# plai-group/latent-flexible-video-diffusion-modeling

Measured on AMD Instinct MI355X. Metric: denoising steps/sec on 20-frame 4x16x16 latents (sampling; training reported alongside), higher is better.
Workload: dtype f32

## Files before the change

### latent-flexible-video-diffusion-modeling_amd/csrc/attention_spatial_fused.hip

```cpp
#include <cstdlib>

#include "common_hip.h"

namespace {

constexpr unsigned kOOBs = 0x40000000u;

__device__ __forceinline__ bool sf_wg(int N, int heads, int& n, int& h) {
    const int L = blockIdx.x;
    const int xcd = L & 7, r = L >> 3;
    const int slot = r / heads;
    h = r - slot * heads;
    n = slot * 8 + xcd;
    return n < N;
}

template <int FP>
__global__ __launch_bounds__(1024) void attn_spatial_fused_kernel(const float* __restrict__ xn, const float* __restrict__ W,
                                                                 const float* __restrict__ bias, float* __restrict__ o,
                                                                 int N, int P, int C, int heads) {
    constexpr int FG = FP / 16;
    constexpr int QLD = FP + 8, VLD = FP + 4;
    extern __shared__ __attribute__((aligned(16))) float sf_smem[];
    int n, h;
    if (!sf_wg(N, heads, n, h)) return;
    const int tid = threadIdx.x, lane = tid & 63;
    const int wave = __builtin_amdgcn_readfirstlane(tid >> 6);
    const int NW = (int)(blockDim.x >> 6);
    const int lq = lane & 15, kk = lane >> 4;
    const int PP = (P + 15) & ~15;
    const int SPR = C >> 2;
    float* Xs = sf_smem;
    float* Ws = Xs + (size_t)PP * C;
    float* Qs = Ws + (size_t)3 * FP * C;
    float* Ks = Qs + (size_t)PP * QLD;
    float* Vs = Ks + (size_t)PP * QLD;

    {
        const __amdgpu_buffer_rsrc_t rsX = __builtin_amdgcn_make_buffer_rsrc((void*)(xn + (size_t)n * P * C), 0, P * C * 4, 0x00020000);
        const __amdgpu_buffer_rsrc_t rsW = __builtin_amdgcn_make_buffer_rsrc((void*)W, 0, 3 * C * C * 4, 0x00020000);
        const int sh = 31 - __builtin_clz(SPR);
        const int nX = (PP * SPR + 63) >> 6, nW = (3 * FP * SPR + 63) >> 6;
        const bool pow2 = (SPR & (SPR - 1)) == 0;
        for (int pc = wave; pc < nX + nW; pc += NW) {
            const bool isX = pc < nX;
            const int ps = (isX ? pc : pc - nX) * 64 + lane;
            int r, s;
            if (pow2) { r = ps >> sh; s = ps & (SPR - 1); }
            else { r = (int)(((float)ps + 0.5f) * __builtin_amdgcn_rcpf((float)SPR)); s = ps - r * SPR; }
            const int ls = (s & ~15) | ((s ^ r) & 15);
            unsigned off;
            if (isX) {
                off = r < P ? (unsigned)(r * C + ls * 4) * 4u : kOOBs;
            } else {
                const int which = r / FP, f = r - which * FP;
                off = r < 3 * FP ? (unsigned)((which * C + h * FP + f) * C + ls * 4) * 4u : kOOBs;
            }
            float* dst = (isX ? Xs : Ws) + (size_t)(isX ? pc : pc - nX) * 256;
            __builtin_amdgcn_raw_ptr_buffer_load_lds(isX ? rsX : rsW, (__attribute__((address_space(3))) void*)dst, 16, (int)off, 0, 0, 0);
        }
    }
    asm volatile("s_waitcnt vmcnt(0)" ::: "memory");
    __syncthreads();

    {
        const float scale = rsqrtf((float)FP) * 1.4426950408889634f;
        const int NRT = PP >> 4;
        const int CG = C >> 4;
        for (int item = wave; item < NRT * FG; item += NW) {
            const int rt = item / FG, fg = item - rt * FG;
            const int xr = 16 * rt + lq;
            const float* xrow = Xs + (size_t)xr * C;
            int wr[3];
            const float* wrow[3];
#pragma unroll
            for (int w = 0; w < 3; ++w) {
                wr[w] = w * FP + 16 * fg + lq;
                wrow[w] = Ws + (size_t)wr[w] * C;
            }
            f32x4 acc[3];
#pragma unroll
            for (int w = 0; w < 3; ++w) acc[w] = (f32x4){0.f, 0.f, 0.f, 0.f};
            for (int g = 0; g < CG; ++g) {
                const int s = 4 * g + kk;
                const f32x4 a4 = ld4(xrow + (((s & ~15) | ((s ^ xr) & 15)) << 2));
                f32x4 b4[3];
#pragma unroll
                for (int w = 0; w < 3; ++w) b4[w] = ld4(wrow[w] + (((s & ~15) | ((s ^ wr[w]) & 15)) << 2));
#pragma unroll
                for (int e = 0; e < 4; ++e)
#pragma unroll
                    for (int w = 0; w < 3; ++w) acc[w] = __builtin_amdgcn_mfma_f32_16x16x4f32(a4[e], b4[w][e], acc[w], 0, 0, 0);
            }
            const int f = 16 * fg + lq;
#pragma unroll
            for (int w = 0; w < 3; ++w) {
                const float bv = bias[w * C + h * FP + f];
                float* dst = w == 0 ? Qs : (w == 1 ? Ks : Vs);
                const int ld = w == 2 ? VLD : QLD;
#pragma unroll
                for (int r = 0; r < 4; ++r) {
                    float v = acc[w][r] + bv;
                    if (w == 0) v *= scale;
                    dst[(size_t)(16 * rt + 4 * kk + r) * ld + f] = v;
                }
            }
        }
    }
    __syncthreads();

    const int NQT = PP >> 4;
    for (int qt = wave; qt < NQT; qt += NW) {
        const int q = 16 * qt + lq;
        f32x4 qf[FG], oacc[FG], oacc2[FG];
#pragma unroll
        for (int g = 0; g < FG; ++g) {
            qf[g] = ld4(Qs + (size_t)q * QLD + 16 * g + 4 * kk);
            oacc[g] = (f32x4){0.f, 0.f, 0.f, 0.f};
            oacc2[g] = (f32x4){0.f, 0.f, 0.f, 0.f};
        }
        float m_run = -INFINITY, l_run = 0.f;
        for (int kb = 0; kb < P; kb += 64) {
            f32x4 s[4];
            int keyr[4];
#pragma unroll
            for (int j = 0; j < 4; ++j) {
                s[j] = (f32x4){0.f, 0.f, 0.f, 0.f};
                keyr[j] = min(kb + 16 * j + lq, PP - 1);
            }
#pragma unroll
            for (int g = 0; g < FG; ++g) {
                f32x4 k4[4];
#pragma unroll
                for (int j = 0; j < 4; ++j) k4[j] = ld4(Ks + (size_t)keyr[j] * QLD + 16 * g + 4 * kk);
#pragma unroll
                for (int e = 0; e < 4; ++e)
#pragma unroll
                    for (int j = 0; j < 4; ++j) s[j] = __builtin_amdgcn_mfma_f32_16x16x4f32(k4[j][e], qf[g][e], s[j], 0, 0, 0);
            }
            float mx = -INFINITY;
            if (kb + 64 > P) {
#pragma unroll
                for (int j = 0; j < 4; ++j)
#pragma unroll
                    for (int r = 0; r < 4; ++r)
                        if (kb + 16 * j + 4 * kk + r >= P) s[j][r] = -INFINITY;
            }
#pragma unroll
            for (int j = 0; j < 4; ++j)
#pragma unroll
                for (int r = 0; r < 4; ++r) mx = fmaxf(mx, s[j][r]);
            mx = fmaxf(mx, __shfl_xor(mx, 16, 64));
            mx = fmaxf(mx, __shfl_xor(mx, 32, 64));
            const float m_new = fmaxf(m_run, mx);
            const float alpha = __builtin_amdgcn_exp2f(m_run - m_new);
            float psum = 0.f;
#pragma unroll
            for (int j = 0; j < 4; ++j)
#pragma unroll
                for (int r = 0; r < 4; ++r) {
                    const float pv = __builtin_amdgcn_exp2f(s[j][r] - m_new);
                    s[j][r] = pv;
                    psum += pv;
                }
            l_run = l_run * alpha + psum;
            m_run = m_new;
#pragma unroll
            for (int g = 0; g < FG; ++g) { oacc[g] *= alpha; oacc2[g] *= alpha; }
#pragma unroll
            for (int j = 0; j < 4; j += 2)
#pragma unroll
                for (int r = 0; r < 4; ++r) {
                    const int key0 = min(kb + 16 * j + 4 * kk + r, PP - 1);
                    const int key1 = min(kb + 16 * (j + 1) + 4 * kk + r, PP - 1);
                    const float* v0 = Vs + (size_t)key0 * VLD + lq;
                    const float* v1 = Vs + (size_t)key1 * VLD + lq;
#pragma unroll
                    for (int g = 0; g < FG; ++g) {
                        oacc[g] = __builtin_amdgcn_mfma_f32_16x16x4f32(v0[16 * g], s[j][r], oacc[g], 0, 0, 0);
                        oacc2[g] = __builtin_amdgcn_mfma_f32_16x16x4f32(v1[16 * g], s[j + 1][r], oacc2[g], 0, 0, 0);
                    }
                }
        }
        l_run += __shfl_xor(l_run, 16, 64);
        l_run += __shfl_xor(l_run, 32, 64);
        const float inv = 1.0f / l_run;
        if (q < P) {
#pragma unroll
            for (int g = 0; g < FG; ++g) st4(o + ((size_t)n * P + q) * C + h * FP + 16 * g + 4 * kk, (oacc[g] + oacc2[g]) * inv);
        }
    }
}

inline size_t sf_lds_bytes(int P, int C, int FP) {
    const size_t PP = (size_t)((P + 15) & ~15);
    const size_t xs = (PP * C + 255) & ~(size_t)255, ws = ((size_t)3 * FP * C + 255) & ~(size_t)255;
    return (xs + ws + 2 * PP * (FP + 8) + PP * (FP + 4)) * sizeof(float);
}

}

extern "C" int lfvdm_attn_spatial_fused_ok(int N, int P, int C, int heads) {
    if (N <= 0 || P <= 0 || heads <= 0 || C % heads) return LFVDM_E_SHAPE;
    const int F = C / heads;
    if ((F != 16 && F != 32 && F != 64) || C % 64) return LFVDM_E_UNSUPPORTED;
    if ((long)P * C * 4 >= (1L << 30) || sf_lds_bytes(P, C, F) > 160 * 1024) return LFVDM_E_UNSUPPORTED;
    return LFVDM_OK;
}

extern "C" int lfvdm_attn_spatial_fused(const float* xn, const float* Wqkv, const float* bqkv, float* o, int N, int P, int C,
                                        int heads, void* stream) {
    if (!xn || !Wqkv || !bqkv || !o) return LFVDM_E_SHAPE;
    if (int rc = lfvdm_attn_spatial_fused_ok(N, P, C, heads)) return rc;
    const int F = C / heads;
    const size_t lds = sf_lds_bytes(P, C, F);
    const unsigned grid = 8u * (unsigned)((N + 7) / 8) * (unsigned)heads;
    const int PP = (P + 15) & ~15, items = (PP / 16) * (F / 16);
    int nw = PP / 16 > items ? PP / 16 : items;
    nw = nw < 4 ? 4 : nw > 16 ? 16 : nw;
    static const int force_nw = getenv("LFVDM_SF_WAVES") ? atoi(getenv("LFVDM_SF_WAVES")) : 0;
    if (force_nw >= 1 && force_nw <= 16) nw = force_nw;
    hipStream_t s = (hipStream_t)stream;
#define LFVDM_SF(FV)                                                                                                         \
    {                                                                                                                        \
        static DynLdsLimit limit;                                                                                            \
        if (int rc = limit.ensure(reinterpret_cast<const void*>(&attn_spatial_fused_kernel<FV>), lds)) return rc;            \
        hipLaunchKernelGGL((attn_spatial_fused_kernel<FV>), dim3(grid), dim3(64 * nw), lds, s, xn, Wqkv, bqkv, o, N, P, C, heads); \
    }
    if (F == 16) LFVDM_SF(16)
    else if (F == 32) LFVDM_SF(32)
    else LFVDM_SF(64)
#undef LFVDM_SF
    LFVDM_CHECK_LAUNCH();
    return LFVDM_OK;
}
```

Baseline: 1231.

## Double-buffer X row chunks in spatial attention QKV projection to overlap loads

The X tile is now staged into LDS in row chunks with two buffers, so the QKV projection of one chunk overlaps the buffer loads of the next, and LDS footprint shrinks. Work items are split per Q/K/V matrix to expose more parallelism, bias values are prefetched into registers, and the K loop is unrolled by four. This adds finer-grained waits and barriers, and changes the wave-count heuristic (minimum of four removed). The extra synchronisation per chunk may cost more than it saves on small spatial sizes.

```diff
diff --git a/latent-flexible-video-diffusion-modeling_amd/csrc/attention_spatial_fused.hip b/latent-flexible-video-diffusion-modeling_amd/csrc/attention_spatial_fused.hip
--- a/latent-flexible-video-diffusion-modeling_amd/csrc/attention_spatial_fused.hip
+++ b/latent-flexible-video-diffusion-modeling_amd/csrc/attention_spatial_fused.hip
@@ -13,6 +13,25 @@
     h = r - slot * heads;
     n = slot * 8 + xcd;
     return n < N;
+}
+
+__host__ __device__ inline int sf_chunk_rows(int C) {
+    const int ch = (4096 / C) & ~15;
+    return ch < 16 ? 16 : ch;
+}
+
+__device__ __forceinline__ void lds_barrier() {
+    asm volatile("s_waitcnt lgkmcnt(0)" ::: "memory");
+    __builtin_amdgcn_s_barrier();
+    asm volatile("" ::: "memory");
+}
+
+__device__ __forceinline__ void sf_wait_vm(int n) {
+    if (n <= 0) asm volatile("s_waitcnt vmcnt(0)" ::: "memory");
+    else if (n == 1) asm volatile("s_waitcnt vmcnt(1)" ::: "memory");
+    else if (n == 2) asm volatile("s_waitcnt vmcnt(2)" ::: "memory");
+    else if (n == 3) asm volatile("s_waitcnt vmcnt(3)" ::: "memory");
+    else asm volatile("s_waitcnt vmcnt(4)" ::: "memory");
 }
 
 template <int FP>
@@ -30,84 +49,110 @@
     const int lq = lane & 15, kk = lane >> 4;
     const int PP = (P + 15) & ~15;
     const int SPR = C >> 2;
+    const int CH = sf_chunk_rows(C);
+    const int NCH = (PP + CH - 1) / CH;
+    const size_t XB = (size_t)CH * C;
     float* Xs = sf_smem;
-    float* Ws = Xs + (size_t)PP * C;
+    float* Ws = Xs + (size_t)(PP < 2 * CH ? PP : 2 * CH) * C;
     float* Qs = Ws + (size_t)3 * FP * C;
     float* Ks = Qs + (size_t)PP * QLD;
     float* Vs = Ks + (size_t)PP * QLD;
 
-    {
-        const __amdgpu_buffer_rsrc_t rsX = __builtin_amdgcn_make_buffer_rsrc((void*)(xn + (size_t)n * P * C), 0, P * C * 4, 0x00020000);
-        const __amdgpu_buffer_rsrc_t rsW = __builtin_amdgcn_make_buffer_rsrc((void*)W, 0, 3 * C * C * 4, 0x00020000);
-        const int sh = 31 - __builtin_clz(SPR);
-        const int nX = (PP * SPR + 63) >> 6, nW = (3 * FP * SPR + 63) >> 6;
-        const bool pow2 = (SPR & (SPR - 1)) == 0;
-        for (int pc = wave; pc < nX + nW; pc += NW) {
-            const bool isX = pc < nX;
-            const int ps = (isX ? pc : pc - nX) * 64 + lane;
+    float bvs[3][FG];
+#pragma unroll
+    for (int w = 0; w < 3; ++w)
+#pragma unroll
+        for (int g = 0; g < FG; ++g)
+            asm volatile("global_load_dword %0, %1, off" : "=&v"(bvs[w][g]) : "v"(bias + w * C + h * FP + 16 * g + lq) : "memory");
+
+    const __amdgpu_buffer_rsrc_t rsX = __builtin_amdgcn_make_buffer_rsrc((void*)(xn + (size_t)n * P * C), 0, P * C * 4, 0x00020000);
+    const int sh = 31 - __builtin_clz(SPR);
+    const bool pow2 = (SPR & (SPR - 1)) == 0;
+    auto chunk_pieces = [&](int c) { return ((PP - c * CH < CH ? PP - c * CH : CH) * SPR) >> 6; };
+    auto my_pieces = [&](int npc) { return wave < npc ? (npc - wave + NW - 1) / NW : 0; };
+    auto stage_chunk = [&](int c) {
+        const int r0 = c * CH, npc = chunk_pieces(c);
+        float* buf = Xs + (size_t)(c & 1) * XB;
+        for (int pc = wave; pc < npc; pc += NW) {
+            const int ps = pc * 64 + lane;
             int r, s;
             if (pow2) { r = ps >> sh; s = ps & (SPR - 1); }
             else { r = (int)(((float)ps + 0.5f) * __builtin_amdgcn_rcpf((float)SPR)); s = ps - r * SPR; }
             const int ls = (s & ~15) | ((s ^ r) & 15);
-            unsigned off;
-            if (isX) {
-                off = r < P ? (unsigned)(r * C + ls * 4) * 4u : kOOBs;
-            } else {
-                const int which = r / FP, f = r - which * FP;
-                off = r < 3 * FP ? (unsigned)((which * C + h * FP + f) * C + ls * 4) * 4u : kOOBs;
-            }
-            float* dst = (isX ? Xs : Ws) + (size_t)(isX ? pc : pc - nX) * 256;
-            __builtin_amdgcn_raw_ptr_buffer_load_lds(isX ? rsX : rsW, (__attribute__((address_space(3))) void*)dst, 16, (int)off, 0, 0, 0);
-        }
-    }
-    asm volatile("s_waitcnt vmcnt(0)" ::: "memory");
-    __syncthreads();
+            const unsigned off = r0 + r < P ? (unsigned)((r0 + r) * C + ls * 4) * 4u : kOOBs;
+            __builtin_amdgcn_raw_ptr_buffer_load_lds(rsX, (__attribute__((address_space(3))) void*)(buf + (size_t)pc * 256), 16, (int)off, 0, 0, 0);
+        }
+    };
+    {
+        const __amdgpu_buffer_rsrc_t rsW = __builtin_amdgcn_make_buffer_rsrc((void*)W, 0, 3 * C * C * 4, 0x00020000);
+        const int nW = (3 * FP * SPR) >> 6;
+        for (int pc = wave; pc < nW; pc += NW) {
+            const int ps = pc * 64 + lane;
+            int r, s;
+            if (pow2) { r = ps >> sh; s = ps & (SPR - 1); }
+            else { r = (int)(((float)ps + 0.5f) * __builtin_amdgcn_rcpf((float)SPR)); s = ps - r * SPR; }
+            const int ls = (s & ~15) | ((s ^ r) & 15);
+            const int which = r / FP, f = r - which * FP;
+            const unsigned off = r < 3 * FP ? (unsigned)((which * C + h * FP + f) * C + ls * 4) * 4u : kOOBs;
+            __builtin_amdgcn_raw_ptr_buffer_load_lds(rsW, (__attribute__((address_space(3))) void*)(Ws + (size_t)pc * 256), 16, (int)off, 0, 0, 0);
+        }
+    }
+    stage_chunk(0);
+    if (NCH > 1) stage_chunk(1);
 
     {
         const float scale = rsqrtf((float)FP) * 1.4426950408889634f;
-        const int NRT = PP >> 4;
         const int CG = C >> 4;
-        for (int item = wave; item < NRT * FG; item += NW) {
-            const int rt = item / FG, fg = item - rt * FG;
-            const int xr = 16 * rt + lq;
-            const float* xrow = Xs + (size_t)xr * C;
-            int wr[3];
-            const float* wrow[3];
-#pragma unroll
-            for (int w = 0; w < 3; ++w) {
-                wr[w] = w * FP + 16 * fg + lq;
-                wrow[w] = Ws + (size_t)wr[w] * C;
-            }
-            f32x4 acc[3];
-#pragma unroll
-            for (int w = 0; w < 3; ++w) acc[w] = (f32x4){0.f, 0.f, 0.f, 0.f};
-            for (int g = 0; g < CG; ++g) {
-                const int s = 4 * g + kk;
-                const f32x4 a4 = ld4(xrow + (((s & ~15) | ((s ^ xr) & 15)) << 2));
-                f32x4 b4[3];
-#pragma unroll
-                for (int w = 0; w < 3; ++w) b4[w] = ld4(wrow[w] + (((s & ~15) | ((s ^ wr[w]) & 15)) << 2));
-#pragma unroll
-                for (int e = 0; e < 4; ++e)
-#pragma unroll
-                    for (int w = 0; w < 3; ++w) acc[w] = __builtin_amdgcn_mfma_f32_16x16x4f32(a4[e], b4[w][e], acc[w], 0, 0, 0);
-            }
-            const int f = 16 * fg + lq;
-#pragma unroll
-            for (int w = 0; w < 3; ++w) {
-                const float bv = bias[w * C + h * FP + f];
+        for (int c = 0; c < NCH; ++c) {
+            sf_wait_vm(c == 0 && NCH > 1 ? my_pieces(chunk_pieces(1)) : 0);
+#pragma unroll
+            for (int w = 0; w < 3; ++w)
+#pragma unroll
+                for (int g = 0; g < FG; ++g) asm volatile("" : "+v"(bvs[w][g]));
+            lds_barrier();
+            if (c >= 1 && c + 1 < NCH) stage_chunk(c + 1);
+            const int rows = PP - c * CH < CH ? PP - c * CH : CH;
+            const float* buf = Xs + (size_t)(c & 1) * XB;
+            for (int item = wave; item < (rows >> 4) * 3 * FG; item += NW) {
+                const int rtl = item / (3 * FG), t = item - rtl * 3 * FG;
+                const int fg = t / 3, w = t - 3 * fg;
+                const int xr = 16 * rtl + lq;
+                const float* xrow = buf + (size_t)xr * C;
+                const int wr = w * FP + 16 * fg + lq;
+                const float* wrow = Ws + (size_t)wr * C;
+                f32x4 acc = (f32x4){0.f, 0.f, 0.f, 0.f};
+                for (int g4 = 0; g4 < CG; g4 += 4) {
+                    f32x4 a4[4], b4[4];
+#pragma unroll
+                    for (int u = 0; u < 4; ++u) {
+                        const int s = 4 * (g4 + u) + kk;
+                        a4[u] = ld4(xrow + (((s & ~15) | ((s ^ xr) & 15)) << 2));
+                        b4[u] = ld4(wrow + (((s & ~15) | ((s ^ wr) & 15)) << 2));
+                    }
+#pragma unroll
+                    for (int u = 0; u < 4; ++u)
+#pragma unroll
+                        for (int e = 0; e < 4; ++e) acc = __builtin_amdgcn_mfma_f32_16x16x4f32(a4[u][e], b4[u][e], acc, 0, 0, 0);
+                }
+                const int f = 16 * fg + lq;
+                float bv = 0.f;
+#pragma unroll
+                for (int w2 = 0; w2 < 3; ++w2)
+#pragma unroll
+                    for (int g2 = 0; g2 < FG; ++g2)
+                        if (w2 == w && g2 == fg) bv = bvs[w2][g2];
                 float* dst = w == 0 ? Qs : (w == 1 ? Ks : Vs);
                 const int ld = w == 2 ? VLD : QLD;
 #pragma unroll
                 for (int r = 0; r < 4; ++r) {
-                    float v = acc[w][r] + bv;
+                    float v = acc[r] + bv;
                     if (w == 0) v *= scale;
-                    dst[(size_t)(16 * rt + 4 * kk + r) * ld + f] = v;
-                }
-            }
-        }
-    }
-    __syncthreads();
+                    dst[(size_t)(c * CH + 16 * rtl + 4 * kk + r) * ld + f] = v;
+                }
+            }
+        }
+    }
+    lds_barrier();
 
     const int NQT = PP >> 4;
     for (int qt = wave; qt < NQT; qt += NW) {
@@ -193,6 +238,12 @@
 }
 
 inline size_t sf_lds_bytes(int P, int C, int FP) {
+    const size_t PP = (size_t)((P + 15) & ~15), CH = (size_t)sf_chunk_rows(C);
+    const size_t xs = (PP < 2 * CH ? PP : 2 * CH) * C, ws = (size_t)3 * FP * C;
+    return (xs + ws + 2 * PP * (FP + 8) + PP * (FP + 4)) * sizeof(float);
+}
+
+inline size_t sf_admit_bytes(int P, int C, int FP) {
     const size_t PP = (size_t)((P + 15) & ~15);
     const size_t xs = (PP * C + 255) & ~(size_t)255, ws = ((size_t)3 * FP * C + 255) & ~(size_t)255;
     return (xs + ws + 2 * PP * (FP + 8) + PP * (FP + 4)) * sizeof(float);
@@ -204,7 +255,7 @@
     if (N <= 0 || P <= 0 || heads <= 0 || C % heads) return LFVDM_E_SHAPE;
     const int F = C / heads;
     if ((F != 16 && F != 32 && F != 64) || C % 64) return LFVDM_E_UNSUPPORTED;
-    if ((long)P * C * 4 >= (1L << 30) || sf_lds_bytes(P, C, F) > 160 * 1024) return LFVDM_E_UNSUPPORTED;
+    if ((long)P * C * 4 >= (1L << 30) || sf_admit_bytes(P, C, F) > 160 * 1024) return LFVDM_E_UNSUPPORTED;
     return LFVDM_OK;
 }
 
@@ -215,9 +266,10 @@
     const int F = C / heads;
     const size_t lds = sf_lds_bytes(P, C, F);
     const unsigned grid = 8u * (unsigned)((N + 7) / 8) * (unsigned)heads;
-    const int PP = (P + 15) & ~15, items = (PP / 16) * (F / 16);
+    const int PP = (P + 15) & ~15, CH = sf_chunk_rows(C);
+    const int items = ((PP < CH ? PP : CH) / 16) * 3 * (F / 16);
     int nw = PP / 16 > items ? PP / 16 : items;
-    nw = nw < 4 ? 4 : nw > 16 ? 16 : nw;
+    nw = nw > 16 ? 16 : nw;
     static const int force_nw = getenv("LFVDM_SF_WAVES") ? atoi(getenv("LFVDM_SF_WAVES")) : 0;
     if (force_nw >= 1 && force_nw <= 16) nw = force_nw;
     hipStream_t s = (hipStream_t)stream;
```

Measured after the change: 1222. About the same (-0.7%).
